# rygorous/ryg_rans

Hardware: AMD Instinct MI355X
Metric: decode GB/s (uncompressed), 64-way interleaved rANS (word format) (higher is better)
Workload: dtype u32; 1 GPU; word format, 64-way interleaved decode of 1024 MiB Zipf(256,s=1) bytes per GPU, 32768-symbol chunks, tables in LDS (BASELINE configs[2]); format=word, n_ways=64, chunk_syms=32768, scale_bits=12, symbols_per_gpu=1073741824

## Files before the change

ryg_rans_amd/csrc/decode_common.hpp:

```cpp
#pragma once

#include "device_common.hpp"
#include "launchers.hpp"

namespace rans_amd {

namespace {

constexpr uint32_t kMaxAdvance = 512;
static_assert(kRingMirror >= kMaxAdvance + 256, "mirror must cover one checkpoint interval plus one sub-step");
constexpr uint32_t kRsrcFlags = 0x00020000u;
constexpr int kAuxNt = 2;

typedef __amdgpu_buffer_rsrc_t rsrc_t;

struct StreamWindow {
    uint8_t *ring;
    uint32_t ring_addr;
    uint32_t cur, mark;
    uint32_t lapped;
    uint32_t gnext;
    rsrc_t rsrc;
    u32x4 pre;

    __device__ __forceinline__ u32x4 fetch(uint32_t lane)
    {
        const u32x4 v = __builtin_amdgcn_raw_buffer_load_b128(rsrc, gnext + lane * 16u, 0, kAuxNt);
        gnext += kRingBlock;
        return v;
    }
    __device__ __forceinline__ void put(uint32_t lane, uint32_t at, const u32x4 &v)
    {
        *reinterpret_cast<u32x4 *>(ring + at + lane * 16u) = v;
        if (at == 0 && lane < kRingMirror / 16u)
            *reinterpret_cast<u32x4 *>(ring + kRingBytes + lane * 16u) = v;
    }
    static __device__ __forceinline__ rsrc_t stream_rsrc(uint64_t chunk_base, uint32_t first, uint32_t fetchable)
    {
        const uint32_t skip = first & ~15u;
        return __builtin_amdgcn_make_buffer_rsrc(reinterpret_cast<void *>(chunk_base + skip), 0, fetchable - skip,
                                                 kRsrcFlags);
    }
    __device__ __forceinline__ void open(uint8_t *lds, uint64_t chunk_base, uint32_t first, uint32_t fetchable,
                                         uint32_t lane)
    {
        const rsrc_t r = stream_rsrc(chunk_base, first, fetchable);
        u32x4 b0, b1;
        prefetch(r, lane, b0, b1);
        install(lds, r, first, lane, b0, b1);
    }
    static __device__ __forceinline__ void prefetch(rsrc_t r, uint32_t lane, u32x4 &b0, u32x4 &b1)
    {
        b0 = __builtin_amdgcn_raw_buffer_load_b128(r, lane * 16u, 0, kAuxNt);
        b1 = __builtin_amdgcn_raw_buffer_load_b128(r, lane * 16u + kRingBlock, 0, kAuxNt);
    }
    __device__ __forceinline__ void install(uint8_t *lds, rsrc_t r, uint32_t first, uint32_t lane, const u32x4 &b0,
                                            const u32x4 &b1)
    {
        ring = lds;
        ring_addr = (uint32_t)(uintptr_t)(__attribute__((address_space(3))) uint8_t *)lds;
        rsrc = r;
        lapped = first & ~15u;
        gnext = 2u * kRingBlock;
        cur = ring_addr + (first & 15u);
        mark = ring_addr + kRingBlock;
        pre = fetch(lane);
        put(lane, 0, b0);
        put(lane, kRingBlock, b1);
    }
    rsrc_t marker_rsrc;
    u32x4 rsrc4;
    template <bool kMarker = false> __device__ __forceinline__ void checkpoint(uint32_t lane)
    {
        if (cur >= mark) {
            if (mark == ring_addr + kRingBlock) {
                put(lane, 0, pre);
                mark = ring_addr + kRingBytes;
            } else {
                cur -= kRingBytes;
                lapped += kRingBytes;
                put(lane, kRingBlock, pre);
                mark = ring_addr + kRingBlock;
            }
            pre = fetch(lane);
            if constexpr (kMarker) {
                __builtin_amdgcn_raw_buffer_store_b32(gnext, marker_rsrc, lane * 4u, 0, 0);
            }
        }
    }
    __device__ __forceinline__ uint32_t cursor() const { return cur - ring_addr; }
    __device__ __forceinline__ void consume(uint32_t bytes) { cur += bytes; }
    __device__ __forceinline__ uint32_t position() const { return lapped + (cur - ring_addr); }
};

template <int FMT>
__device__ __forceinline__ uint32_t dec_renorm(const StreamWindow &W, typename FmtTraits<FMT>::state_t &x,
                                               bool active)
{
    if constexpr (kIsWord<FMT>) {
        const bool need = active && x < (1u << 16);
        const uint64_t m = __builtin_amdgcn_ballot_w64(need);
        const uint32_t at = W.cursor() + 2u * rank_below(m);
        const uint32_t w = *reinterpret_cast<const uint16_t *>(W.ring + at);
        x = need ? ((x << 16) | w) : x;
        return 2u * (uint32_t)__builtin_popcountll(m);
    } else if constexpr (kIsR64<FMT>) {
        const bool need = active && x < (1ull << 31);
        const uint64_t m = __builtin_amdgcn_ballot_w64(need);
        const uint32_t at = W.cursor() + 4u * rank_below(m);
        const uint32_t w = *reinterpret_cast<const uint32_t *>(W.ring + at);
        x = need ? ((x << 32) | w) : x;
        return 4u * (uint32_t)__builtin_popcountll(m);
    } else {
        const bool n1 = active && x < (1u << 23);
        const bool n2 = active && x < (1u << 15);
        const uint64_t m1 = __builtin_amdgcn_ballot_w64(n1);
        const uint64_t m2 = __builtin_amdgcn_ballot_w64(n2);
        const uint32_t at = W.cursor() + rank_below(m1) + rank_below(m2);
        const uint32_t b0 = W.ring[at];
        const uint32_t b1 = W.ring[at + 1];
        const uint32_t x1 = (x << 8) | b0;
        const uint32_t x2 = (x1 << 8) | b1;
        x = n2 ? x2 : (n1 ? x1 : x);
        return (uint32_t)__builtin_popcountll(m1) + (uint32_t)__builtin_popcountll(m2);
    }
}

__device__ __forceinline__ void renorm_word_full(uint32_t &x, uint32_t &cur, uint32_t k65536)
{
    uint32_t t, w, cnt;
    asm volatile("v_cmpx_gt_u32_e32 vcc, %[lim], %[x]\n\t"
                 "s_bcnt1_i32_b64 %[cnt], vcc\n\t"
                 "s_nop 0\n\t"
                 "v_mbcnt_lo_u32_b32 %[t], vcc_lo, 0\n\t"
                 "v_mbcnt_hi_u32_b32 %[t], vcc_hi, %[t]\n\t"
                 "v_lshl_add_u32 %[t], %[t], 1, %[cur]\n\t"
                 "ds_read_u16 %[w], %[t]\n\t"
                 "s_lshl1_add_u32 %[cur], %[cnt], %[cur]\n\t"
                 "s_waitcnt lgkmcnt(0)\n\t"
                 "v_perm_b32 %[x], %[x], %[w], %[sel]\n\t"
                 "s_mov_b64 exec, -1"
                 : [x] "+v"(x), [t] "=&v"(t), [w] "=&v"(w), [cnt] "=&s"(cnt), [cur] "+s"(cur)
                 : [lim] "v"(k65536), [sel] "s"(0x05040100u)
                 : "vcc", "scc", "memory");
}

__device__ __forceinline__ void renorm_byte_full(uint32_t &x, uint32_t &cur, uint32_t k2p23, uint32_t k2p15)
{
    uint32_t t, b0, b1, c1, c2;
    asm volatile("v_cmp_gt_u32_e64 s[52:53], %[l23], %[x]\n\t"
                 "v_cmp_gt_u32_e32 vcc, %[l15], %[x]\n\t"
                 "s_bcnt1_i32_b64 %[c1], s[52:53]\n\t"
                 "v_mbcnt_lo_u32_b32 %[t], s52, 0\n\t"
                 "v_mbcnt_hi_u32_b32 %[t], s53, %[t]\n\t"
                 "s_bcnt1_i32_b64 %[c2], vcc\n\t"
                 "v_mbcnt_lo_u32_b32 %[t], vcc_lo, %[t]\n\t"
                 "v_mbcnt_hi_u32_b32 %[t], vcc_hi, %[t]\n\t"
                 "v_add_u32_e32 %[t], %[cur], %[t]\n\t"
                 "s_add_i32 %[cur], %[cur], %[c1]\n\t"
                 "s_mov_b64 exec, s[52:53]\n\t"
                 "ds_read_u8 %[b0], %[t]\n\t"
                 "ds_read_u8 %[b1], %[t] offset:1\n\t"
                 "s_add_i32 %[cur], %[cur], %[c2]\n\t"
                 "s_waitcnt lgkmcnt(0)\n\t"
                 "v_lshl_or_b32 %[x], %[x], 8, %[b0]\n\t"
                 "s_mov_b64 exec, vcc\n\t"
                 "v_lshl_or_b32 %[x], %[x], 8, %[b1]\n\t"
                 "s_mov_b64 exec, -1"
                 : [x] "+v"(x), [t] "=&v"(t), [b0] "=&v"(b0), [b1] "=&v"(b1), [c1] "=&s"(c1), [c2] "=&s"(c2), [cur] "+s"(cur)
                 : [l23] "v"(k2p23), [l15] "v"(k2p15)
                 : "vcc", "scc", "memory", "s52", "s53");
}

#define RANS_STORE_MODS " nt sc1"
constexpr int kAuxStore = 2 | 16;

__device__ __forceinline__ rsrc_t marker_rsrc(const DecParams &p, uint32_t wave_in_grid)
{
    return __builtin_amdgcn_make_buffer_rsrc(
        reinterpret_cast<void *>(uniform64(reinterpret_cast<uint64_t>(p.wave_scratch) + (uint64_t)uniform(wave_in_grid) * 64u)),
        0, p.wave_scratch ? 4u : 0u, kRsrcFlags);
}

__device__ __forceinline__ void record_span(const DecParams &p, unsigned long long t_start, uint8_t *smem, uint32_t tid)
{
    if (!p.span)
        return;
    unsigned long long *ends = reinterpret_cast<unsigned long long *>(smem);
    __syncthreads();
    if ((tid & 63u) == 0)
        ends[tid >> 6] = wall_clock64();
    __syncthreads();
    if (tid == 0) {
        unsigned long long last = 0;
        for (uint32_t w = 0; w < (blockDim.x >> 6); ++w)
            last = ends[w] > last ? ends[w] : last;
        atomicMax(p.span, ~t_start);
        atomicMax(p.span + 1, last);
    }
}
__device__ __forceinline__ void record_span(const DecParams &p, unsigned long long t_start, uint8_t *smem)
{
    record_span(p, t_start, smem, threadIdx.x);
}

template <int SYMBYTE, int J> __device__ __forceinline__ uint32_t acc_symbol(uint32_t raw, uint32_t acc)
{
    if constexpr (J == 0) {
        return raw;
    } else if constexpr (J == 1) {
        constexpr uint32_t sel = (uint32_t)SYMBYTE | ((4u + SYMBYTE) << 8) | 0x03020000u;
        return __builtin_amdgcn_perm(raw, acc, sel);
    } else {
        constexpr uint32_t ident = 0x03020100u;
        constexpr uint32_t sel = (ident & ~(0xffu << (8 * J))) | ((4u + SYMBYTE) << (8 * J));
        return __builtin_amdgcn_perm(raw, acc, sel);
    }
}

}

}
```

ryg_rans_amd/csrc/decode_wave.hip:

```cpp

#include "decode_common.hpp"

namespace rans_amd {

namespace {

#define RANS_WORD_RENORM                                   \
    "v_cmpx_gt_u32_e32 vcc, %[lim], %[x]\n\t"              \
    "s_bcnt1_i32_b64 %[cnt], vcc\n\t"                      \
    "s_nop 0\n\t"                                          \
    "v_mbcnt_lo_u32_b32 v56, vcc_lo, 0\n\t"                \
    "v_mbcnt_hi_u32_b32 v56, vcc_hi, v56\n\t"              \
    "v_lshl_add_u32 v56, v56, 1, %[cur]\n\t"               \
    "ds_read_u16 v57, v56\n\t"                             \
    "s_lshl1_add_u32 %[cur], %[cnt], %[cur]\n\t"           \
    "s_waitcnt lgkmcnt(0)\n\t"                             \
    "v_perm_b32 %[x], %[x], v57, %[selm]\n\t"              \
    "s_mov_b64 exec, -1\n\t"
#define RANS_WORD_LOOKUP(E)                                \
    "v_and_b32_e32 v56, %[m12], %[x]\n\t"                  \
    "v_lshlrev_b32_e32 v56, 3, v56\n\t"                    \
    "ds_read_b64 " E ", v56\n\t"                           \
    "v_lshrrev_b32_e32 v57, 12, %[x]\n\t"

template <bool kStorePrev>
__device__ __forceinline__ void decode_group_word(uint32_t &x, uint32_t &pa, uint32_t &cur, uint32_t m12,
                                                  uint32_t k65536, uint32_t sel1, uint32_t sel2, uint32_t selA,
                                                  uint32_t selB, uint32_t selC, u32x4 orsrc, uint32_t out_lane_off,
                                                  uint32_t osoff_prev)
{
    uint32_t cnt;
    if constexpr (kStorePrev) {
        asm volatile(
            RANS_WORD_LOOKUP("v[58:59]")
            "v_mov_b32_dpp v60, %[pa] quad_perm:[1,0,3,2] row_mask:0xf bank_mask:0xf\n\t"
            "v_perm_b32 v61, v60, %[pa], %[sel1]\n\t"
            "s_waitcnt lgkmcnt(0)\n\t"
            "v_mad_u32_u24 %[x], v58, v57, v59\n\t"
            "v_mov_b32_dpp v60, v61 quad_perm:[2,3,0,1] row_mask:0xf bank_mask:0xf\n\t"
            "v_perm_b32 v62, v60, v61, %[sel2]\n\t"
            "buffer_store_dword v62, %[ooff], %[orsrc], %[osoff] offen" RANS_STORE_MODS "\n\t"
            RANS_WORD_RENORM
            RANS_WORD_LOOKUP("v[60:61]")
            "s_waitcnt lgkmcnt(0)\n\t"
            "v_mad_u32_u24 %[x], v60, v57, v61\n\t"
            "v_perm_b32 %[pa], v60, v58, %[selA]\n\t"
            RANS_WORD_RENORM
            RANS_WORD_LOOKUP("v[58:59]")
            "s_waitcnt lgkmcnt(0)\n\t"
            "v_mad_u32_u24 %[x], v58, v57, v59\n\t"
            "v_perm_b32 %[pa], v58, %[pa], %[selB]\n\t"
            RANS_WORD_RENORM
            RANS_WORD_LOOKUP("v[60:61]")
            "s_waitcnt lgkmcnt(0)\n\t"
            "v_mad_u32_u24 %[x], v60, v57, v61\n\t"
            "v_perm_b32 %[pa], v60, %[pa], %[selC]\n\t"
            RANS_WORD_RENORM
            : [x] "+v"(x), [pa] "+v"(pa), [cur] "+s"(cur), [cnt] "=&s"(cnt)
            : [m12] "v"(m12), [lim] "v"(k65536), [sel1] "v"(sel1), [sel2] "v"(sel2), [selA] "v"(selA), [selB] "v"(selB),
              [selC] "v"(selC), [selm] "s"(0x05040100u), [orsrc] "s"(orsrc), [ooff] "v"(out_lane_off),
              [osoff] "s"(osoff_prev)
            : "vcc", "scc", "memory", "v56", "v57", "v58", "v59", "v60", "v61", "v62"
            );
    } else {
        asm volatile(
            RANS_WORD_LOOKUP("v[58:59]")
            "s_waitcnt lgkmcnt(0)\n\t"
            "v_mad_u32_u24 %[x], v58, v57, v59\n\t"
            RANS_WORD_RENORM
            RANS_WORD_LOOKUP("v[60:61]")
            "s_waitcnt lgkmcnt(0)\n\t"
            "v_mad_u32_u24 %[x], v60, v57, v61\n\t"
            "v_perm_b32 %[pa], v60, v58, %[selA]\n\t"
            RANS_WORD_RENORM
            RANS_WORD_LOOKUP("v[58:59]")
            "s_waitcnt lgkmcnt(0)\n\t"
            "v_mad_u32_u24 %[x], v58, v57, v59\n\t"
            "v_perm_b32 %[pa], v58, %[pa], %[selB]\n\t"
            RANS_WORD_RENORM
            RANS_WORD_LOOKUP("v[60:61]")
            "s_waitcnt lgkmcnt(0)\n\t"
            "v_mad_u32_u24 %[x], v60, v57, v61\n\t"
            "v_perm_b32 %[pa], v60, %[pa], %[selC]\n\t"
            RANS_WORD_RENORM
            : [x] "+v"(x), [pa] "+v"(pa), [cur] "+s"(cur), [cnt] "=&s"(cnt)
            : [m12] "v"(m12), [lim] "v"(k65536), [selA] "v"(selA), [selB] "v"(selB), [selC] "v"(selC),
              [selm] "s"(0x05040100u)
            : "vcc", "scc", "memory", "v56", "v57", "v58", "v59", "v60", "v61", "v62"
            );
    }
}
#undef RANS_WORD_RENORM
#undef RANS_WORD_LOOKUP


template <int FMT, int K, int OUT, bool RAGGED = false>
__global__ void __launch_bounds__(kDecBlockThreads, (K <= 2 ? 8 : 4)) k_decode(const DecParams p)
{
    using Tr = FmtTraits<FMT>;
    using state_t = typename Tr::state_t;
    extern __shared__ __attribute__((aligned(16))) uint8_t smem[];
    const unsigned long long t_start = (p.trace || p.span) ? wall_clock64() : 0ull;
    const unsigned long long c_start = p.trace ? __builtin_readcyclecounter() : 0ull;
    uint32_t rounds_done = 0;

    const uint32_t t0_bytes = kIsAdaptive<FMT> ? (blockDim.x >> 6) * kAdaptDecWaveLds : (p.table0_bytes + 15u) & ~15u;
    const uint32_t t1_bytes = kIsAdaptive<FMT> ? 0u : (p.table1_bytes + 15u) & ~15u;
    if constexpr (!kIsAdaptive<FMT>) {
        const uint4 *g0 = reinterpret_cast<const uint4 *>(p.table0);
        uint4 *l0 = reinterpret_cast<uint4 *>(smem);
        for (uint32_t i = threadIdx.x; i < t0_bytes / 16u; i += blockDim.x)
            l0[i] = g0[i];
        const uint4 *g1 = reinterpret_cast<const uint4 *>(p.table1);
        uint4 *l1 = reinterpret_cast<uint4 *>(smem + t0_bytes);
        for (uint32_t i = threadIdx.x; i < t1_bytes / 16u; i += blockDim.x)
            l1[i] = g1[i];
    }
    __syncthreads();

    const uint32_t lane = lane_id();
    const uint32_t wave = uniform(threadIdx.x >> 6);
    const uint32_t waves_per_block = blockDim.x >> 6;

    DecTables<FMT> T;
    if constexpr (kIsAdaptive<FMT>)
        T.init(smem + wave * kAdaptDecWaveLds, smem + wave * kAdaptDecWaveLds + (1u << kAdaptMaxScaleBits), p.scale_bits,
               p.log2nsyms);
    else
        T.init(smem, smem + t0_bytes, p.scale_bits, p.log2nsyms);
    if (!lds_starts_at_zero(smem)) {
        if (threadIdx.x == 0)
            atomicAdd(p.err_count, 1ull << 32);
        return;
    }

    uint8_t *ring = smem + t0_bytes + t1_bytes + wave * kRingStride;
    const uint32_t N = (OUT != OUT_SLOW) ? 64u * K : p.n_ways;
    const uint64_t cbase = reinterpret_cast<uint64_t>(p.container);

    const uint32_t sel1 = (lane & 1u) ? 0x03070105u : 0x06020400u;
    const uint32_t sel2 = (lane & 2u) ? 0x03020706u : 0x05040100u;
    const uint32_t out_lane_off = (lane & 3u) * N + (lane & ~3u);

    if (p.work_counter_reset && blockIdx.x == 0 && threadIdx.x < kWorkPools)
        p.work_counter_reset[threadIdx.x * kWorkPoolStride] = 0u;
    if (p.span_reset && blockIdx.x == 0 && threadIdx.x < 2)
        p.span_reset[threadIdx.x] = 0ull;
    const uint64_t total_waves = (uint64_t)gridDim.x * waves_per_block;
    uint64_t chunk_v = (uint64_t)blockIdx.x * waves_per_block + wave;
    const uint32_t npools = gridDim.x < kWorkPools ? gridDim.x : kWorkPools;
    const uint32_t pool = blockIdx.x % npools;
    for (;;) {
        if (p.work_counter) {
            uint32_t got = 0;
            if (lane == 0)
                got = atomicAdd(p.work_counter + pool * kWorkPoolStride, 1u);
            chunk_v = (uint64_t)uniform(got) * npools + pool;
        }
        if (chunk_v >= p.nchunks)
            break;
        uint64_t chunk = uniform64(chunk_v);
        chunk_v += total_waves;
        uint64_t first = chunk * p.chunk_syms;
        uint32_t nsym = 0;
        if constexpr (RAGGED) {
            bool inside = true;
            if (p.order) {
                chunk = uniform64((uint64_t)p.order[chunk]);
                inside = chunk < p.nchunks;
            }
            if (inside) {
                first = uniform64(p.sym_offsets[chunk]);
                nsym = uniform(p.sym_counts[chunk]);
                inside = first <= p.out_syms && nsym <= p.out_syms - first;
            }
            if (!inside) {
                if (lane == 0)
                    atomicAdd(p.err_count, 1ull);
                continue;
            }
        } else {
            nsym = (uint32_t)((p.n - first) < p.chunk_syms ? (p.n - first) : p.chunk_syms);
        }
        const uint64_t off = uniform64(p.offsets[chunk]);
        const uint32_t len = uniform(p.lengths[chunk]);
        const uint64_t src = cbase + off;
        uint8_t RANS_GLOBAL *dst = reinterpret_cast<uint8_t RANS_GLOBAL *>(
            reinterpret_cast<uint64_t>(p.out) + first * p.sym_bytes);

        bool ok = ((off & (Tr::kUnit - 1u)) == 0) && (len >= N * Tr::kStateBytes) && (off <= p.container_bytes) &&
                  (len <= p.container_bytes - off);
        if (!ok) {
            if (lane == 0)
                atomicAdd(p.err_count, 1ull);
            continue;
        }

        if constexpr (kIsAdaptive<FMT>) {
            bool has_row = true;
            if constexpr (RAGGED)
                has_row = nsym != 0;
            if (has_row && !adapt_build_dec(p.chunk_freqs + chunk * 256u, p.scale_bits, lane, const_cast<uint8_t *>(T.t0),
                                 reinterpret_cast<uint32_t *>(const_cast<uint8_t *>(T.t1)))) {
                if (lane == 0)
                    atomicAdd(p.err_count, 1ull);
                continue;
            }
        }

        state_t x[K];
#pragma unroll
        for (int k = 0; k < K; ++k) {
            const uint32_t idx = k * 64u + lane;
            x[k] = Tr::kL;
            if (idx < N) {
                if constexpr (kIsR64<FMT>) {
                    const u32x2 v = *(reinterpret_cast<const u32x2 RANS_GLOBAL *>(src) + idx);
                    x[k] = (uint64_t)v.x | ((uint64_t)v.y << 32);
                } else {
                    x[k] = *(reinterpret_cast<const uint32_t RANS_GLOBAL *>(src) + idx);
                }
            }
        }

        StreamWindow W;
        const uint32_t skip = (uint32_t)off & 15u;
        const uint64_t room = ((p.container_bytes + 15u) & ~uint64_t(15)) - (off - skip);
        const uint32_t climit = (skip + len + 15u) & ~15u;
        W.open(ring, src - skip, skip + N * Tr::kStateBytes, climit < room ? climit : (uint32_t)room, lane);

        const uint32_t rounds = uniform(nsym / N);
        rounds_done += rounds;
        const uint32_t tail = uniform(nsym - rounds * N);
        uint32_t r = 0;
        bool dword_out = true;
        if constexpr (RAGGED)
            dword_out = (uniform((uint32_t)reinterpret_cast<uint64_t>(dst)) & 3u) == 0;
        constexpr int kCheckEvery = kIsR64<FMT> ? 2 : 4;

        if constexpr (OUT == OUT_FAST16) {
            const uint32_t pairs = dword_out ? rounds >> 1 : 0u;
            uint8_t RANS_GLOBAL *gdst = dst;
            const uint32_t sel16 = (lane & 1u) ? 0x03020706u : 0x05040100u;
            const uint32_t lane_off16 = ((lane & 1u) * N + (lane & ~1u)) * 2u;
            const uint32_t k2p23 = (1u << 23) + (lane >> 6), k2p15 = (1u << 15) + (lane >> 6);
            const uint32_t k65536w = 0x10000u + (lane >> 6);
            for (uint32_t g = 0; g < pairs; ++g) {
                uint32_t acc[K];
#pragma unroll
                for (int J = 0; J < 2; ++J) {
#pragma unroll
                    for (int k = 0; k < K; ++k) {
                        const uint32_t s16 = dec_step<FMT>(T, x[k]) & 0xffffu;
                        acc[k] = J == 0 ? s16 : (acc[k] | (s16 << 16));
                    }
#pragma unroll
                    for (int k = 0; k < K; ++k) {
                        if ((J * K + k) % kCheckEvery == 0)
                            W.checkpoint(lane);
                        if constexpr (kIsByteStream<FMT>)
                            renorm_byte_full(x[k], W.cur, k2p23, k2p15);
                        else if constexpr (FMT == FMT_WORD16)
                            renorm_word_full(x[k], W.cur, k65536w);
                        else
                            W.consume(dec_renorm<FMT>(W, x[k], true));
                    }
                }
#pragma unroll
                for (int k = 0; k < K; ++k) {
                    const uint32_t o = quad_perm<1, 0, 3, 2>(acc[k]);
                    const uint32_t v = __builtin_amdgcn_perm(o, acc[k], sel16);
                    __builtin_nontemporal_store(v, reinterpret_cast<uint32_t RANS_GLOBAL *>(gdst + (lane_off16 + k * 128u)));
                }
                gdst += 4u * N;
            }
            r = pairs << 1;
        } else if constexpr (OUT != OUT_SLOW) {
            const uint32_t groups = dword_out ? rounds >> 2 : 0u;
            const rsrc_t orsrc = __builtin_amdgcn_make_buffer_rsrc(
                reinterpret_cast<void *>(reinterpret_cast<uint64_t>(dst)), 0, nsym, kRsrcFlags);
            uint32_t osoff = 0;
            const uint32_t k65536 = 0x10000u + (lane >> 6);
            const uint32_t k2p23 = (1u << 23) + (lane >> 6), k2p15 = (1u << 15) + (lane >> 6);
            for (uint32_t g = 0; g < groups; ++g) {
                uint32_t acc[K];
#define RANS_ROUND(J)                                                              \
    _Pragma("unroll") for (int k = 0; k < K; ++k)                                  \
        acc[k] = acc_symbol<Tr::kSymByte, J>(dec_step<FMT>(T, x[k]), acc[k]);      \
    _Pragma("unroll") for (int k = 0; k < K; ++k) {                                \
        if ((J * K + k) % kCheckEvery == 0)                                        \
            W.checkpoint(lane);                                                    \
        if constexpr (FMT == FMT_WORD || FMT == FMT_WORDA)                         \
            renorm_word_full(x[k], W.cur, k65536);                                 \
        else if constexpr (kIsByteStream<FMT>)                                     \
            renorm_byte_full(x[k], W.cur, k2p23, k2p15);                           \
        else                                                                       \
            W.consume(dec_renorm<FMT>(W, x[k], true));                             \
    }
                RANS_ROUND(0)
                RANS_ROUND(1)
                RANS_ROUND(2)
                RANS_ROUND(3)
#undef RANS_ROUND
                if constexpr (K == 1)
                    W.checkpoint(lane);
#pragma unroll
                for (int k = 0; k < K; ++k) {
                    const uint32_t v = quad_transpose(acc[k], sel1, sel2);
                    __builtin_amdgcn_raw_buffer_store_b32(v, orsrc, out_lane_off + k * 64u, osoff, kAuxStore);
                }
                osoff += 4u * N;
            }
            r = groups << 2;
        }

        for (; r <= rounds; ++r) {
            const uint32_t cnt = (r < rounds) ? N : tail;
            if (cnt == 0)
                break;
            uint8_t RANS_GLOBAL *rdst = dst + (uint64_t)r * N * p.sym_bytes;
#pragma unroll
            for (int k = 0; k < K; ++k) {
                const uint32_t idx = k * 64u + lane;
                if (idx < cnt) {
                    uint32_t s = dec_step<FMT>(T, x[k]);
                    if constexpr (Tr::kSymByte == 3)
                        s >>= 24;
                    if (p.sym_bytes == 1)
                        rdst[idx] = (uint8_t)s;
                    else
                        reinterpret_cast<uint16_t RANS_GLOBAL *>(rdst)[idx] = (uint16_t)s;
                }
            }
#pragma unroll
            for (int k = 0; k < K; ++k) {
                const uint32_t idx = k * 64u + lane;
                W.checkpoint(lane);
                W.consume(dec_renorm<FMT>(W, x[k], idx < cnt));
            }
        }

        bool good = true;
#pragma unroll
        for (int k = 0; k < K; ++k)
            good = good && (x[k] == Tr::kL);
        const bool all_good = __builtin_amdgcn_ballot_w64(!good) == 0 && W.position() == skip + len;
        if (!all_good && lane == 0)
            atomicAdd(p.err_count, 1ull);
    }
    if (p.trace && lane == 0) {
        unsigned long long *t = p.trace + (uint64_t)kTraceWords * ((uint64_t)blockIdx.x * waves_per_block + wave);
        t[0] = t_start;
        t[1] = wall_clock64();
        t[2] = __builtin_amdgcn_s_getreg((20 ) | (0 << 6) | ((4 - 1) << 11));
        t[3] = __builtin_readcyclecounter() - c_start;
        t[4] = rounds_done;
    }
    record_span(p, t_start, smem);
}

constexpr uint32_t kClaimAhead = 10, kDataAhead = 5;

__device__ __forceinline__ rsrc_t chunk_rsrc(uint64_t cbase, uint64_t cbytes16, uint64_t off, uint32_t len)
{
    off = uniform64(off);
    len = uniform(len);
    const uint32_t skip = (uint32_t)off & 15u;
    const uint64_t room = cbytes16 - (off - skip);
    const uint32_t climit = (skip + len + 15u) & ~15u;
    return StreamWindow::stream_rsrc(cbase + (off - skip), skip + 64u * 4u, climit < room ? climit : (uint32_t)room);
}

constexpr int kWord64Threads = kDecBlockThreads;
template <bool RAGGED>
__global__ void __launch_bounds__(kWord64Threads, 8) k_decode_word64_t(const DecParams p)
{
    using Tr = FmtTraits<FMT_WORD>;
    constexpr uint32_t N = 64;
    extern __shared__ __attribute__((aligned(16))) uint8_t smem[];
    const unsigned long long t_start = (p.trace || p.span) ? wall_clock64() : 0ull;
    const unsigned long long c_start = p.trace ? __builtin_readcyclecounter() : 0ull;
    uint32_t rounds_done = 0;

    const uint32_t t0_bytes = (p.table0_bytes + 15u) & ~15u;
    {
        const uint4 *g0 = reinterpret_cast<const uint4 *>(p.table0);
        uint4 *l0 = reinterpret_cast<uint4 *>(smem);
        for (uint32_t i = threadIdx.x; i < t0_bytes / 16u; i += blockDim.x)
            l0[i] = g0[i];
    }
    __syncthreads();

    const uint32_t lane = lane_id();
    const uint32_t wave = uniform(threadIdx.x >> 6);
    const uint32_t waves_per_block = blockDim.x >> 6;
    DecTables<FMT_WORD> T;
    T.init(smem, smem + t0_bytes, p.scale_bits, p.log2nsyms);
    if (!lds_starts_at_zero(smem)) {
        if (threadIdx.x == 0)
            atomicAdd(p.err_count, 1ull << 32);
        return;
    }
    uint8_t *ring = smem + t0_bytes + wave * kRingStride;
    const uint64_t cbase = reinterpret_cast<uint64_t>(p.container);
    const uint64_t cbytes16 = (p.container_bytes + 15u) & ~uint64_t(15);

    const uint32_t sel1 = (lane & 1u) ? 0x03070105u : 0x06020400u;
    const uint32_t sel2 = (lane & 2u) ? 0x03020706u : 0x05040100u;
    const uint32_t out_lane_off = (lane & 3u) * N + (lane & ~3u);
    uint32_t selA = 0x03020703u, selB = 0x03070100u, selC = 0x07020100u;
    uint32_t k65536 = 0x10000u, m12 = 0xfffu;
    asm volatile("v_mov_b32 %0, %0" : "+v"(selA));
    asm volatile("v_mov_b32 %0, %0" : "+v"(selB));
    asm volatile("v_mov_b32 %0, %0" : "+v"(selC));
    asm volatile("v_mov_b32 %0, %0" : "+v"(k65536));
    asm volatile("v_mov_b32 %0, %0" : "+v"(m12));

    if (p.work_counter_reset && blockIdx.x == 0 && threadIdx.x < kWorkPools)
        p.work_counter_reset[threadIdx.x * kWorkPoolStride] = 0u;
    if (p.span_reset && blockIdx.x == 0 && threadIdx.x < 2)
        p.span_reset[threadIdx.x] = 0ull;
    if constexpr (!RAGGED)
        if (p.word64_counters_reset && blockIdx.x == 0 && threadIdx.x < kWord64Pools)
            p.word64_counters_reset[threadIdx.x * kWorkPoolStride] = 0u;

    constexpr uint32_t kPools = RAGGED ? kWorkPools : kWord64Pools;
    unsigned int *const counters = RAGGED ? p.work_counter : p.word64_counters;
    const uint64_t total_waves = (uint64_t)gridDim.x * waves_per_block;
    uint64_t static_next = (uint64_t)blockIdx.x * waves_per_block + wave;
    const uint32_t npools = gridDim.x < kPools ? gridDim.x : kPools;
    const uint32_t pool = blockIdx.x % npools;
    uint32_t claimed_v = 0;

    uint64_t n_idx = 0;
    uint64_t n_off = 0;
    uint32_t n_len = 0;
    uint64_t n_first = 0;
    uint32_t n_nsym = 0;
    uint32_t n_x = 0;
    u32x4 n_b0 = {0u, 0u, 0u, 0u}, n_b1 = n_b0;
    bool n_any = false, n_ok = false;

#define RANS_STEP_CLAIM()                                                                   \
    do {                                                                                    \
        if (counters && lane == 0)                                                          \
            claimed_v = atomicAdd(counters + pool * kWorkPoolStride, 1u);                   \
    } while (0)
#define RANS_STEP_DATA()                                                                    \
    do {                                                                                    \
        if (counters) {                                                                     \
            n_idx = (uint64_t)uniform(claimed_v) * npools + pool;                           \
        } else {                                                                            \
            n_idx = uniform64(static_next);                                                 \
            static_next += total_waves;                                                     \
        }                                                                                   \
        n_any = n_idx < p.nchunks;                                                          \
        n_ok = false;                                                                       \
        if (n_any) {                                                                        \
            if constexpr (RAGGED) {                                                         \
                bool n_inside = true;                                                       \
                if (p.order) {  \
                    uint32_t n_ord;                                                         \
                    asm volatile("s_load_dword %0, %1, 0x0\n\ts_waitcnt lgkmcnt(0)"         \
                                 : "=&s"(n_ord)                                             \
                                 : "s"(uniform64(reinterpret_cast<uint64_t>(p.order + n_idx))) \
                                 : "memory");                                               \
                    n_idx = uniform64((uint64_t)uniform(n_ord));                            \
                    n_inside = n_idx < p.nchunks;                                           \
                }                                                                           \
                if (n_inside) {      \
                    asm volatile("s_load_dwordx2 %0, %4, 0x0\n\ts_load_dword %1, %5, 0x0\n\t" \
                                 "s_load_dwordx2 %2, %6, 0x0\n\ts_load_dword %3, %7, 0x0\n\ts_waitcnt lgkmcnt(0)" \
                                 : "=&s"(n_off), "=&s"(n_len), "=&s"(n_first), "=&s"(n_nsym) \
                                 : "s"(uniform64(reinterpret_cast<uint64_t>(p.offsets + n_idx))), \
                                   "s"(uniform64(reinterpret_cast<uint64_t>(p.lengths + n_idx))), \
                                   "s"(uniform64(reinterpret_cast<uint64_t>(p.sym_offsets + n_idx))), \
                                   "s"(uniform64(reinterpret_cast<uint64_t>(p.sym_counts + n_idx))) \
                                 : "memory");                                               \
                    n_off = uniform64(n_off);                                               \
                    n_len = uniform(n_len);                                                 \
                    n_first = uniform64(n_first);                                           \
                    n_nsym = uniform(n_nsym);                                               \
                    n_inside = n_first <= p.out_syms && n_nsym <= p.out_syms - n_first;     \
                }                                                                           \
                n_ok = n_inside && ((n_off & 1u) == 0) && (n_len >= N * Tr::kStateBytes) && (n_off <= p.container_bytes) && \
                       (n_len <= p.container_bytes - n_off);                                \
            } else {                                                                        \
            asm volatile("s_load_dwordx2 %0, %2, 0x0\n\ts_load_dword %1, %3, 0x0\n\ts_waitcnt lgkmcnt(0)" \
                         : "=&s"(n_off), "=&s"(n_len)                                       \
                         : "s"(uniform64(reinterpret_cast<uint64_t>(p.offsets + n_idx))),   \
                           "s"(uniform64(reinterpret_cast<uint64_t>(p.lengths + n_idx)))    \
                         : "memory");                                                       \
            n_off = uniform64(n_off);  \
            n_len = uniform(n_len);                                                         \
            n_ok = ((n_off & 1u) == 0) && (n_len >= N * Tr::kStateBytes) && (n_off <= p.container_bytes) && \
                   (n_len <= p.container_bytes - n_off);                                    \
            }                                                                               \
            if (n_ok) {                                                                     \
                n_x = *(reinterpret_cast<const uint32_t RANS_GLOBAL *>(cbase + n_off) + lane); \
                StreamWindow::prefetch(chunk_rsrc(cbase, cbytes16, n_off, n_len), lane, n_b0, n_b1); \
            } else if (lane == 0) {                                                         \
                atomicAdd(p.err_count, 1ull);                                               \
            }                                                                               \
        }                                                                                   \
    } while (0)

    for (;;) {
        RANS_STEP_CLAIM();
        RANS_STEP_DATA();
        if (n_ok || !n_any)
            break;
    }
    while (n_ok) {
        const uint64_t c_idx = uniform64(n_idx);
        const uint32_t c_skip = uniform((uint32_t)n_off & 15u);
        const uint32_t c_len = uniform(n_len) + c_skip;
        StreamWindow W;
        W.install(ring, chunk_rsrc(cbase, cbytes16, n_off, n_len), c_skip + N * Tr::kStateBytes, lane, n_b0, n_b1);
        uint32_t x = n_x;
        const uint64_t first_sym = RAGGED ? uniform64(n_first) : c_idx * p.chunk_syms;
        const uint32_t nsym = RAGGED ? uniform(n_nsym)
                                     : uniform((uint32_t)((p.n - first_sym) < p.chunk_syms ? (p.n - first_sym) : p.chunk_syms));
        uint8_t RANS_GLOBAL *dst = reinterpret_cast<uint8_t RANS_GLOBAL *>(reinterpret_cast<uint64_t>(p.out) + first_sym);
        const uint32_t rounds = uniform(nsym / N);
        const uint32_t tail = uniform(nsym - rounds * N);
        const uint32_t groups = (!RAGGED || (uniform((uint32_t)reinterpret_cast<uint64_t>(dst)) & 3u) == 0) ? rounds >> 2 : 0u;
        rounds_done += rounds;
        n_any = false;
        n_ok = false;
        uint32_t stage = 0;

        if (groups) {
            const uint64_t dsta = reinterpret_cast<uint64_t>(dst);
            const u32x4 orsrc = {uniform((uint32_t)dsta), uniform((uint32_t)(dsta >> 32)) & 0xffffu,
                                 uniform(nsym), kRsrcFlags};
            uint32_t pa = 0;
            W.marker_rsrc = marker_rsrc(p, blockIdx.x * waves_per_block + wave);
            W.template checkpoint<true>(lane);
            decode_group_word<false>(x, pa, W.cur, m12, k65536, sel1, sel2, selA, selB, selC, orsrc, out_lane_off, 0u);
            const uint32_t oend = (groups - 1u) * 256u;
            uint32_t trigger = groups > kClaimAhead ? (groups - kClaimAhead) * 256u : 0u;
            for (uint32_t osoff = 0; osoff != oend; osoff += 256u) {
                if (osoff == trigger) {
                    if (stage == 0) {
                        RANS_STEP_CLAIM();
                        trigger += (kClaimAhead - kDataAhead) * 256u;
                    } else {
                        RANS_STEP_DATA();
                        trigger = ~0u;
                    }
                    ++stage;
                }
                W.template checkpoint<true>(lane);
                decode_group_word<true>(x, pa, W.cur, m12, k65536, sel1, sel2, selA, selB, selC, orsrc, out_lane_off, osoff);
            }
            const uint32_t v = quad_transpose(pa, sel1, sel2);
            __builtin_nontemporal_store(v, reinterpret_cast<uint32_t RANS_GLOBAL *>(dst + oend + out_lane_off));
        }
        if (stage < 1)
            RANS_STEP_CLAIM();
        if (stage < 2)
            RANS_STEP_DATA();

        for (uint32_t r = groups << 2; r <= rounds; ++r) {
            const uint32_t cnt = (r < rounds) ? N : tail;
            if (cnt == 0)
                break;
            if (lane < cnt) {
                const uint32_t sy = dec_step<FMT_WORD>(T, x);
                dst[(uint64_t)r * N + lane] = (uint8_t)(sy >> 24);
            }
            W.checkpoint(lane);
            W.consume(dec_renorm<FMT_WORD>(W, x, lane < cnt));
        }

        const bool all_good = __builtin_amdgcn_ballot_w64(x != Tr::kL) == 0 && W.position() == c_len;
        if (!all_good && lane == 0)
            atomicAdd(p.err_count, 1ull);

        while (n_any && !n_ok) {
            RANS_STEP_CLAIM();
            RANS_STEP_DATA();
        }
    }
#undef RANS_STEP_CLAIM
#undef RANS_STEP_DATA
    if (p.trace && lane == 0) {
        unsigned long long *t = p.trace + (uint64_t)kTraceWords * ((uint64_t)blockIdx.x * waves_per_block + wave);
        t[0] = t_start;
        t[1] = wall_clock64();
        t[2] = __builtin_amdgcn_s_getreg((20 ) | (0 << 6) | ((4 - 1) << 11));
        t[3] = __builtin_readcyclecounter() - c_start;
        t[4] = rounds_done;
    }
    record_span(p, t_start, smem);
}

template <int FMT, int K, int OUT, bool RAGGED> hipError_t launch_decode_t(const WaveLaunch &g, hipStream_t stream, const DecParams &p)
{
    if constexpr (decode_is_word64(FMT, K, OUT))
        return launch_wave_kernel<k_decode_word64_t<RAGGED>>(g, kCuLdsBytes, stream, p);
    else if constexpr (decode_has(FMT, K, OUT, RAGGED))
        return launch_wave_kernel<k_decode<FMT, K, OUT, RAGGED>>(g, kCuLdsBytes, stream, p);
    else
        return hipErrorInvalidValue;
}

template <int FMT, bool RAGGED> hipError_t launch_decode_f(const DecParams &p, int num_cus, hipStream_t stream, KernelId *name)
{
    const bool aligned = decode_out_aligned(FMT, reinterpret_cast<uintptr_t>(p.out), p.chunk_syms);
    const DecodeShape s = decode_shape(FMT, p.n_ways, p.sym_bytes, aligned, RAGGED);
    const WaveLaunch g = decode_launch(s.word64, kIsAdaptive<FMT>, p.table0_bytes, p.table1_bytes, p.nchunks, num_cus);
    if (!s.K || !g.threads)
        return hipErrorInvalidValue;
    if (kIsAdaptive<FMT> && (!p.chunk_freqs || p.scale_bits > kAdaptMaxScaleBits || p.scale_bits < 8 || (FMT == FMT_WORDA && p.scale_bits != 12)))
        return hipErrorInvalidValue;
    if (name)
        *name = s.word64 ? KernelId::decode_word64
                : FMT == FMT_WORD ? KernelId::decode_word : FMT == FMT_BYTE ? KernelId::decode_byte : FMT == FMT_BYTEF ? KernelId::decode_byte_slot_records
                : FMT == FMT_R64 ? KernelId::decode_r64 : FMT == FMT_R64S ? KernelId::decode_r64_search
                : FMT == FMT_WORD16 ? KernelId::decode_word_u16
                : FMT == FMT_BYTEA ? KernelId::decode_byte_chunk_models : FMT == FMT_WORDA ? KernelId::decode_word_chunk_models : KernelId::decode_alias;
    return with_states_per_lane(s.K, [&](auto k) {
        constexpr int K = decltype(k)::value;
        switch (s.out) {
        case OUT_FAST8: return launch_decode_t<FMT, K, OUT_FAST8, RAGGED>(g, stream, p);
        case OUT_FAST16: return launch_decode_t<FMT, K, OUT_FAST16, RAGGED>(g, stream, p);
        default: return launch_decode_t<FMT, K, OUT_SLOW, RAGGED>(g, stream, p);
        }
    });
}

template <bool RAGGED> hipError_t launch_decode_fmt(int format, const DecParams &p, int num_cus, hipStream_t stream, KernelId *name)
{
    switch (format) {
    case FMT_WORD: return launch_decode_f<FMT_WORD, RAGGED>(p, num_cus, stream, name);
    case FMT_BYTE: return launch_decode_f<FMT_BYTE, RAGGED>(p, num_cus, stream, name);
    case FMT_BYTEF: return launch_decode_f<FMT_BYTEF, RAGGED>(p, num_cus, stream, name);
    case FMT_R64: return launch_decode_f<FMT_R64, RAGGED>(p, num_cus, stream, name);
    case FMT_R64S: return launch_decode_f<FMT_R64S, RAGGED>(p, num_cus, stream, name);
    case FMT_WORD16: return launch_decode_f<FMT_WORD16, RAGGED>(p, num_cus, stream, name);
    case FMT_BYTEA: return launch_decode_f<FMT_BYTEA, RAGGED>(p, num_cus, stream, name);
    case FMT_WORDA: return launch_decode_f<FMT_WORDA, RAGGED>(p, num_cus, stream, name);
    case FMT_ALIAS: return launch_decode_f<FMT_ALIAS, RAGGED>(p, num_cus, stream, name);
    default: return hipErrorInvalidValue;
    }
}

}

hipError_t launch_decode_batch_wave(int format, const DecParams &p, int num_cus, hipStream_t stream, KernelId *name)
{
    if (!p.sym_offsets || !p.sym_counts)
        return hipErrorInvalidValue;
    const bool word64 = format == FMT_WORD && p.n_ways == 64 && p.sym_bytes == 1;
    if (name)
        *name = word64                 ? KernelId::decode_batch_word64
                : format == FMT_WORD   ? KernelId::decode_batch_word
                : format == FMT_BYTE   ? KernelId::decode_batch_byte
                : format == FMT_BYTEF  ? KernelId::decode_batch_byte_slot_records
                : format == FMT_R64    ? KernelId::decode_batch_r64
                : format == FMT_R64S   ? KernelId::decode_batch_r64_search
                : format == FMT_WORD16 ? KernelId::decode_batch_word_u16
                                       : KernelId::decode_batch_alias;
    if (format == FMT_BYTEA || format == FMT_WORDA)
        return hipErrorInvalidValue;
    return launch_decode_fmt<true>(format, p, num_cus, stream, nullptr);
}

hipError_t launch_decode_batch_models_wave(int format, const DecParams &p, int num_cus, hipStream_t stream, KernelId *name)
{
    if (!p.sym_offsets || !p.sym_counts || p.sym_bytes != 1)
        return hipErrorInvalidValue;
    switch (format) {
    case FMT_WORDA:
        if (name)
            *name = KernelId::decode_batch_models_word;
        return launch_decode_f<FMT_WORDA, true>(p, num_cus, stream, nullptr);
    case FMT_BYTEA:
        if (name)
            *name = KernelId::decode_batch_models_byte;
        return launch_decode_f<FMT_BYTEA, true>(p, num_cus, stream, nullptr);
    default: return hipErrorInvalidValue;
    }
}

hipError_t launch_decode_wave(int format, const DecParams &p, int num_cus, hipStream_t stream, KernelId *name)
{
    return launch_decode_fmt<false>(format, p, num_cus, stream, name);
}

}
```

Before: 2817 GB/s.

## Replace StreamWindow with hand-scheduled Word64Window using pinned VGPRs and vmcnt ladders

Introduces a dedicated ring-buffer window for the 64-way word decoder that issues chunk prefetches and ring refills into fixed, reserved VGPRs through inline asm. It waits with precise vmcnt counts computed from how many groups have elapsed since each load, rather than relying on compiler-inserted waits. It also drops the per-checkpoint debug marker store and caps the compiler at 44 VGPRs. The goal is to cut wait stalls and register and store overhead in the hot loop. The cost is fragile hand-managed register reservation and counter bookkeeping that must stay consistent with every load issued.

Measured after the change: 2822 GB/s, median of 2. About the same (+0.2%).

```diff
diff --git a/ryg_rans_amd/csrc/decode_common.hpp b/ryg_rans_amd/csrc/decode_common.hpp
--- a/ryg_rans_amd/csrc/decode_common.hpp
+++ b/ryg_rans_amd/csrc/decode_common.hpp
@@ -68,9 +68,8 @@
         put(lane, 0, b0);
         put(lane, kRingBlock, b1);
     }
-    rsrc_t marker_rsrc;
     u32x4 rsrc4;
-    template <bool kMarker = false> __device__ __forceinline__ void checkpoint(uint32_t lane)
+    __device__ __forceinline__ void checkpoint(uint32_t lane)
     {
         if (cur >= mark) {
             if (mark == ring_addr + kRingBlock) {
@@ -83,9 +82,6 @@
                 mark = ring_addr + kRingBlock;
             }
             pre = fetch(lane);
-            if constexpr (kMarker) {
-                __builtin_amdgcn_raw_buffer_store_b32(gnext, marker_rsrc, lane * 4u, 0, 0);
-            }
         }
     }
     __device__ __forceinline__ uint32_t cursor() const { return cur - ring_addr; }
@@ -175,13 +171,6 @@
 #define RANS_STORE_MODS " nt sc1"
 constexpr int kAuxStore = 2 | 16;
 
-__device__ __forceinline__ rsrc_t marker_rsrc(const DecParams &p, uint32_t wave_in_grid)
-{
-    return __builtin_amdgcn_make_buffer_rsrc(
-        reinterpret_cast<void *>(uniform64(reinterpret_cast<uint64_t>(p.wave_scratch) + (uint64_t)uniform(wave_in_grid) * 64u)),
-        0, p.wave_scratch ? 4u : 0u, kRsrcFlags);
-}
-
 __device__ __forceinline__ void record_span(const DecParams &p, unsigned long long t_start, uint8_t *smem, uint32_t tid)
 {
     if (!p.span)
diff --git a/ryg_rans_amd/csrc/decode_wave.hip b/ryg_rans_amd/csrc/decode_wave.hip
--- a/ryg_rans_amd/csrc/decode_wave.hip
+++ b/ryg_rans_amd/csrc/decode_wave.hip
@@ -361,19 +361,131 @@
 
 constexpr uint32_t kClaimAhead = 10, kDataAhead = 5;
 
-__device__ __forceinline__ rsrc_t chunk_rsrc(uint64_t cbase, uint64_t cbytes16, uint64_t off, uint32_t len)
+__device__ __forceinline__ u32x4 chunk_rsrc(uint64_t cbase, uint64_t cbytes16, uint64_t off, uint32_t len)
 {
     off = uniform64(off);
     len = uniform(len);
     const uint32_t skip = (uint32_t)off & 15u;
     const uint64_t room = cbytes16 - (off - skip);
     const uint32_t climit = (skip + len + 15u) & ~15u;
-    return StreamWindow::stream_rsrc(cbase + (off - skip), skip + 64u * 4u, climit < room ? climit : (uint32_t)room);
-}
+    const uint32_t fetchable = ((uint32_t)(room >> 32) == 0 && (uint32_t)room < climit) ? (uint32_t)room : climit;
+    const uint64_t base = cbase + (off - skip) + 64u * 4u;
+    return u32x4{(uint32_t)base, (uint32_t)(base >> 32) & 0xffffu, fetchable - 64u * 4u, kRsrcFlags};
+}
+
+__device__ __forceinline__ bool less64(uint64_t a, uint64_t b)
+{
+    const uint32_t ah = (uint32_t)(a >> 32), bh = (uint32_t)(b >> 32);
+    return ah < bh || (ah == bh && (uint32_t)a < (uint32_t)b);
+}
+__device__ __forceinline__ bool less_equal64(uint64_t a, uint64_t b) { return !less64(b, a); }
+
+static_assert(kRingBlock == 1024 && kRingBytes == 2048 && kRingMirror == 768, "the offsets and the mirror's exec mask in Word64Window's asm");
+constexpr int kWord64CompilerVgprs = 44;
+#define RANS_W64_REQUEST_REGS "v44", "v45", "v46", "v47", "v48", "v49", "v50", "v51", "v52", "v53", "v54", "v55", "v63"
+#define RANS_VMCNT_LADDER(k)                                                                                  \
+    switch (k) {                                                                                              \
+    case 0: asm volatile("s_waitcnt vmcnt(0)" : : : "memory", RANS_W64_REQUEST_REGS); break;                  \
+    case 1: asm volatile("s_waitcnt vmcnt(1)" : : : "memory", RANS_W64_REQUEST_REGS); break;                  \
+    case 2: asm volatile("s_waitcnt vmcnt(2)" : : : "memory", RANS_W64_REQUEST_REGS); break;                  \
+    case 3: asm volatile("s_waitcnt vmcnt(3)" : : : "memory", RANS_W64_REQUEST_REGS); break;                  \
+    case 4: asm volatile("s_waitcnt vmcnt(4)" : : : "memory", RANS_W64_REQUEST_REGS); break;                  \
+    case 5: asm volatile("s_waitcnt vmcnt(5)" : : : "memory", RANS_W64_REQUEST_REGS); break;                  \
+    case 6: asm volatile("s_waitcnt vmcnt(6)" : : : "memory", RANS_W64_REQUEST_REGS); break;                  \
+    default: asm volatile("s_waitcnt vmcnt(7)" : : : "memory", RANS_W64_REQUEST_REGS); break;                 \
+    }
+#define RANS_RING_PUT_LOW(B)                               \
+    "ds_write_b128 %[wr], " B "\n\t"                       \
+    "s_mov_b32 exec_hi, 0xffff\n\t"                        \
+    "ds_write_b128 %[wr], " B " offset:2048\n\t"           \
+    "s_mov_b32 exec_hi, -1\n\t"
+
+struct Word64Window {
+    uint8_t *ring;
+    uint32_t ring_addr;
+    uint32_t cur, mark;
+    uint32_t lapped;
+    uint32_t wr;
+    uint32_t voff;
+    u32x4 rsrc;
+
+    __device__ __forceinline__ void bind(uint8_t *lds, uint32_t lane)
+    {
+        ring = lds;
+        ring_addr = uniform((uint32_t)(uintptr_t)(__attribute__((address_space(3))) uint8_t *)lds);
+        wr = ring_addr + lane * 16u;
+    }
+    __device__ __forceinline__ void request_chunk(const u32x4 &r, uint64_t states) const
+    {
+        asm volatile("v_subrev_u32_e32 v56, %[ra], %[wr]\n\t"
+                     "v_lshrrev_b32_e32 v57, 2, v56\n\t"
+                     "s_nop 3\n\t"
+                     "global_load_dword v63, v57, %[st]\n\t"
+                     "buffer_load_dwordx4 v[48:51], v56, %[rsrc], 0 offen nt\n\t"
+                     "buffer_load_dwordx4 v[52:55], v56, %[rsrc], 0 offen offset:1024 nt"
+                     :
+                     : [wr] "v"(wr), [ra] "s"(ring_addr), [st] "s"(states), [rsrc] "s"(r)
+                     : "memory", "v56", "v57", RANS_W64_REQUEST_REGS);
+    }
+    __device__ __forceinline__ void install(const u32x4 &r, uint32_t skip, uint32_t k, uint32_t &x)
+    {
+        rsrc = r;
+        lapped = 64u * 4u;
+        cur = ring_addr + skip;
+        mark = ring_addr + kRingBlock;
+        asm volatile("v_subrev_u32_e32 v56, %[ra], %[wr]\n\t"
+                     "s_nop 3\n\t"
+                     "buffer_load_dwordx4 v[44:47], v56, %[rsrc], 0 offen offset:2048 nt\n\t"
+                     "v_add_u32_e32 %[voff], 0xc00, v56"
+                     : [voff] "=&v"(voff)
+                     : [wr] "v"(wr), [ra] "s"(ring_addr), [rsrc] "s"(rsrc)
+                     : "memory", "v56", RANS_W64_REQUEST_REGS);
+        const uint32_t k1 = k + 1u;
+        RANS_VMCNT_LADDER(k1)
+        asm volatile("v_mov_b32_e32 %[x], v63\n\t"
+                     RANS_RING_PUT_LOW("v[48:51]")
+                     "ds_write_b128 %[wr], v[52:55] offset:1024"
+                     : [x] "=&v"(x)
+                     : [wr] "v"(wr)
+                     : "memory", RANS_W64_REQUEST_REGS);
+    }
+    __device__ __forceinline__ bool due() const { return cur >= mark; }
+    __device__ __forceinline__ void refill(uint32_t k)
+    {
+        RANS_VMCNT_LADDER(k)
+        const bool low = mark == ring_addr + kRingBlock;
+        const uint32_t at = low ? 0u : kRingBlock;
+        const uint64_t mirror = low ? (1ull << (kRingMirror / 16u)) - 1ull : 0ull;
+        asm volatile("v_add_u32_e32 v56, %[at], %[wr]\n\t"
+                     "ds_write_b128 v56, v[44:47]\n\t"
+                     "s_mov_b64 exec, %[mirror]\n\t"
+                     "ds_write_b128 v56, v[44:47] offset:2048\n\t"
+                     "s_mov_b64 exec, -1\n\t"
+                     "buffer_load_dwordx4 v[44:47], %[voff], %[rsrc], 0 offen nt\n\t"
+                     "v_add_u32_e32 %[voff], 0x400, %[voff]"
+                     : [voff] "+v"(voff)
+                     : [wr] "v"(wr), [at] "s"(at), [mirror] "s"(mirror), [rsrc] "s"(rsrc)
+                     : "memory", "v56", RANS_W64_REQUEST_REGS);
+        cur = low ? cur : cur - kRingBytes;
+        lapped = low ? lapped : lapped + kRingBytes;
+        mark = ring_addr + (low ? kRingBytes : kRingBlock);
+    }
+    __device__ __forceinline__ uint32_t renorm(uint32_t &x, bool active) const
+    {
+        const bool need = active && x < (1u << 16);
+        const uint64_t m = __builtin_amdgcn_ballot_w64(need);
+        const uint32_t w = *reinterpret_cast<const uint16_t *>(ring + (cur - ring_addr) + 2u * rank_below(m));
+        x = need ? ((x << 16) | w) : x;
+        return 2u * (uint32_t)__builtin_popcountll(m);
+    }
+    __device__ __forceinline__ uint32_t position() const { return lapped + (cur - ring_addr); }
+};
+#undef RANS_RING_PUT_LOW
 
 constexpr int kWord64Threads = kDecBlockThreads;
 template <bool RAGGED>
-__global__ void __launch_bounds__(kWord64Threads, 8) k_decode_word64_t(const DecParams p)
+__global__ void __launch_bounds__(kWord64Threads, 8) __attribute__((amdgpu_num_vgpr(kWord64CompilerVgprs)))
+k_decode_word64_t(const DecParams p)
 {
     using Tr = FmtTraits<FMT_WORD>;
     constexpr uint32_t N = 64;
@@ -401,7 +513,8 @@
             atomicAdd(p.err_count, 1ull << 32);
         return;
     }
-    uint8_t *ring = smem + t0_bytes + wave * kRingStride;
+    Word64Window W0;
+    W0.bind(smem + t0_bytes + wave * kRingStride, lane);
     const uint64_t cbase = reinterpret_cast<uint64_t>(p.container);
     const uint64_t cbytes16 = (p.container_bytes + 15u) & ~uint64_t(15);
 
@@ -429,7 +542,7 @@
     const uint64_t total_waves = (uint64_t)gridDim.x * waves_per_block;
     uint64_t static_next = (uint64_t)blockIdx.x * waves_per_block + wave;
     const uint32_t npools = gridDim.x < kPools ? gridDim.x : kPools;
-    const uint32_t pool = blockIdx.x % npools;
+    const uint32_t pool = uniform(blockIdx.x % npools);
     uint32_t claimed_v = 0;
 
     uint64_t n_idx = 0;
@@ -437,8 +550,6 @@
     uint32_t n_len = 0;
     uint64_t n_first = 0;
     uint32_t n_nsym = 0;
-    uint32_t n_x = 0;
-    u32x4 n_b0 = {0u, 0u, 0u, 0u}, n_b1 = n_b0;
     bool n_any = false, n_ok = false;
 
 #define RANS_STEP_CLAIM()                                                                   \
@@ -452,9 +563,9 @@
             n_idx = (uint64_t)uniform(claimed_v) * npools + pool;                           \
         } else {                                                                            \
             n_idx = uniform64(static_next);                                                 \
-            static_next += total_waves;                                                     \
+            static_next = uniform64(static_next + total_waves);                             \
         }                                                                                   \
-        n_any = n_idx < p.nchunks;                                                          \
+        n_any = less64(n_idx, p.nchunks);                                                   \
         n_ok = false;                                                                       \
         if (n_any) {                                                                        \
             if constexpr (RAGGED) {                                                         \
@@ -466,7 +577,7 @@
                                  : "s"(uniform64(reinterpret_cast<uint64_t>(p.order + n_idx))) \
                                  : "memory");                                               \
                     n_idx = uniform64((uint64_t)uniform(n_ord));                            \
-                    n_inside = n_idx < p.nchunks;                                           \
+                    n_inside = less64(n_idx, p.nchunks);                                    \
                 }                                                                           \
                 if (n_inside) {      \
                     asm volatile("s_load_dwordx2 %0, %4, 0x0\n\ts_load_dword %1, %5, 0x0\n\t" \
@@ -481,10 +592,10 @@
                     n_len = uniform(n_len);                                                 \
                     n_first = uniform64(n_first);                                           \
                     n_nsym = uniform(n_nsym);                                               \
-                    n_inside = n_first <= p.out_syms && n_nsym <= p.out_syms - n_first;     \
+                    n_inside = less_equal64(n_first, p.out_syms) && less_equal64(n_nsym, p.out_syms - n_first); \
                 }                                                                           \
-                n_ok = n_inside && ((n_off & 1u) == 0) && (n_len >= N * Tr::kStateBytes) && (n_off <= p.container_bytes) && \
-                       (n_len <= p.container_bytes - n_off);                                \
+                n_ok = n_inside && ((n_off & 1u) == 0) && (n_len >= N * Tr::kStateBytes) && less_equal64(n_off, p.container_bytes) && \
+                       less_equal64(n_len, p.container_bytes - n_off);                      \
             } else {                                                                        \
             asm volatile("s_load_dwordx2 %0, %2, 0x0\n\ts_load_dword %1, %3, 0x0\n\ts_waitcnt lgkmcnt(0)" \
                          : "=&s"(n_off), "=&s"(n_len)                                       \
@@ -493,12 +604,11 @@
                          : "memory");                                                       \
             n_off = uniform64(n_off);  \
             n_len = uniform(n_len);                                                         \
-            n_ok = ((n_off & 1u) == 0) && (n_len >= N * Tr::kStateBytes) && (n_off <= p.container_bytes) && \
-                   (n_len <= p.container_bytes - n_off);                                    \
+            n_ok = ((n_off & 1u) == 0) && (n_len >= N * Tr::kStateBytes) && less_equal64(n_off, p.container_bytes) && \
+                   less_equal64(n_len, p.container_bytes - n_off);                          \
             }                                                                               \
             if (n_ok) {                                                                     \
-                n_x = *(reinterpret_cast<const uint32_t RANS_GLOBAL *>(cbase + n_off) + lane); \
-                StreamWindow::prefetch(chunk_rsrc(cbase, cbytes16, n_off, n_len), lane, n_b0, n_b1); \
+                W0.request_chunk(chunk_rsrc(cbase, cbytes16, n_off, n_len), uniform64(cbase + n_off)); \
             } else if (lane == 0) {                                                         \
                 atomicAdd(p.err_count, 1ull);                                               \
             }                                                                               \
@@ -511,35 +621,43 @@
         if (n_ok || !n_any)
             break;
     }
+    uint32_t n_behind = 0;
     while (n_ok) {
         const uint64_t c_idx = uniform64(n_idx);
         const uint32_t c_skip = uniform((uint32_t)n_off & 15u);
         const uint32_t c_len = uniform(n_len) + c_skip;
-        StreamWindow W;
-        W.install(ring, chunk_rsrc(cbase, cbytes16, n_off, n_len), c_skip + N * Tr::kStateBytes, lane, n_b0, n_b1);
-        uint32_t x = n_x;
-        const uint64_t first_sym = RAGGED ? uniform64(n_first) : c_idx * p.chunk_syms;
-        const uint32_t nsym = RAGGED ? uniform(n_nsym)
-                                     : uniform((uint32_t)((p.n - first_sym) < p.chunk_syms ? (p.n - first_sym) : p.chunk_syms));
-        uint8_t RANS_GLOBAL *dst = reinterpret_cast<uint8_t RANS_GLOBAL *>(reinterpret_cast<uint64_t>(p.out) + first_sym);
+        Word64Window W = W0;
+        uint32_t x;
+        W.install(chunk_rsrc(cbase, cbytes16, n_off, n_len), c_skip, n_behind, x);
+        uint64_t first_sym;
+        uint32_t nsym;
+        if constexpr (RAGGED) {
+            first_sym = uniform64(n_first);
+            nsym = uniform(n_nsym);
+        } else {
+            first_sym = uniform64(c_idx * p.chunk_syms);
+            const uint64_t left = uniform64(p.n - first_sym);
+            nsym = uniform(less64(left, p.chunk_syms) ? (uint32_t)left : p.chunk_syms);
+        }
+        const uint64_t dsta = uniform64(reinterpret_cast<uint64_t>(p.out) + first_sym);
+        uint8_t RANS_GLOBAL *dst = reinterpret_cast<uint8_t RANS_GLOBAL *>(dsta);
         const uint32_t rounds = uniform(nsym / N);
         const uint32_t tail = uniform(nsym - rounds * N);
-        const uint32_t groups = (!RAGGED || (uniform((uint32_t)reinterpret_cast<uint64_t>(dst)) & 3u) == 0) ? rounds >> 2 : 0u;
+        const uint32_t groups = (!RAGGED || ((uint32_t)dsta & 3u) == 0) ? rounds >> 2 : 0u;
         rounds_done += rounds;
         n_any = false;
         n_ok = false;
+        n_behind = 0;
         uint32_t stage = 0;
+        uint32_t pre_behind = 0;
 
         if (groups) {
-            const uint64_t dsta = reinterpret_cast<uint64_t>(dst);
-            const u32x4 orsrc = {uniform((uint32_t)dsta), uniform((uint32_t)(dsta >> 32)) & 0xffffu,
-                                 uniform(nsym), kRsrcFlags};
+            const u32x4 orsrc = {uniform((uint32_t)dsta), uniform((uint32_t)(dsta >> 32)) & 0xffffu, uniform(nsym), kRsrcFlags};
             uint32_t pa = 0;
-            W.marker_rsrc = marker_rsrc(p, blockIdx.x * waves_per_block + wave);
-            W.template checkpoint<true>(lane);
             decode_group_word<false>(x, pa, W.cur, m12, k65536, sel1, sel2, selA, selB, selC, orsrc, out_lane_off, 0u);
             const uint32_t oend = (groups - 1u) * 256u;
             uint32_t trigger = groups > kClaimAhead ? (groups - kClaimAhead) * 256u : 0u;
+            uint32_t refill_at = 0, data_at = 0;
             for (uint32_t osoff = 0; osoff != oend; osoff += 256u) {
                 if (osoff == trigger) {
                     if (stage == 0) {
@@ -547,15 +665,22 @@
                         trigger += (kClaimAhead - kDataAhead) * 256u;
                     } else {
                         RANS_STEP_DATA();
+                        data_at = osoff;
                         trigger = ~0u;
                     }
                     ++stage;
                 }
-                W.template checkpoint<true>(lane);
+                if (W.due()) {
+                    W.refill((osoff - refill_at) >> 8);
+                    refill_at = osoff;
+                }
                 decode_group_word<true>(x, pa, W.cur, m12, k65536, sel1, sel2, selA, selB, selC, orsrc, out_lane_off, osoff);
             }
             const uint32_t v = quad_transpose(pa, sel1, sel2);
             __builtin_nontemporal_store(v, reinterpret_cast<uint32_t RANS_GLOBAL *>(dst + oend + out_lane_off));
+            pre_behind = ((oend - refill_at) >> 8) + 1u;
+            if (stage == 2)
+                n_behind = ((oend - data_at) >> 8) + 1u;
         }
         if (stage < 1)
             RANS_STEP_CLAIM();
@@ -570,8 +695,11 @@
                 const uint32_t sy = dec_step<FMT_WORD>(T, x);
                 dst[(uint64_t)r * N + lane] = (uint8_t)(sy >> 24);
             }
-            W.checkpoint(lane);
-            W.consume(dec_renorm<FMT_WORD>(W, x, lane < cnt));
+            if (W.due()) {
+                W.refill(pre_behind);
+                pre_behind = 0;
+            }
+            W.cur += W.renorm(x, lane < cnt);
         }
 
         const bool all_good = __builtin_amdgcn_ballot_w64(x != Tr::kL) == 0 && W.position() == c_len;
@@ -581,6 +709,7 @@
         while (n_any && !n_ok) {
             RANS_STEP_CLAIM();
             RANS_STEP_DATA();
+            n_behind = 0;
         }
     }
 #undef RANS_STEP_CLAIM
```
